# AsherBond/0-kno-vectorx

Measured on AMD Instinct MI355X. Metric: header_range_256 proofs/sec, higher is better.
Workload: dtype u64 (Goldilocks) / u8 (hashes)

## Files before the change

0-kno-vectorx_amd/csrc/vx_core.hip:

```cpp
#include <stdarg.h>
#include <stdlib.h>
#include <stdio.h>

#include "gl.cuh"
#include <dlfcn.h>

#include "vx_internal.h"

__attribute__((constructor)) static void vx_runtime_env() { setenv("GPU_MAX_HW_QUEUES", "16", 0); }

int32_t vx_fail(vx_ctx* ctx, int32_t code, const char* fmt, ...) {
    char buf[512];
    va_list ap;
    va_start(ap, fmt);
    vsnprintf(buf, sizeof buf, fmt, ap);
    va_end(ap);
    if (ctx) ctx->err = buf;
    return code;
}

static int32_t make_powtab(vx_ctx* ctx, uint64_t base, PowTab* out) {
    std::vector<uint64_t> h(3 * 2048);
    uint64_t b = base;
    for (int l = 0; l < 3; ++l) {
        uint64_t acc = 1;
        for (int j = 0; j < 2048; ++j) {
            h[l * 2048 + j] = acc;
            acc = glh::mul(acc, b);
        }
        b = glh::pow(b, 2048);
    }
    VX_HIP(hipMalloc(&out->d, h.size() * 8));
    VX_HIP(hipMemcpyAsync(out->d, h.data(), h.size() * 8, hipMemcpyHostToDevice, ctx->stream));
    VX_HIP(hipStreamSynchronize(ctx->stream));
    return VX_OK;
}

int32_t vx_get_shift_tab(vx_ctx* ctx, uint64_t base, PowTab* out) {
    auto it = ctx->shift_tabs.find(base);
    if (it == ctx->shift_tabs.end()) {
        PowTab t;
        VX_TRY(make_powtab(ctx, base, &t));
        it = ctx->shift_tabs.emplace(base, t).first;
    }
    *out = it->second;
    return VX_OK;
}

int32_t vx_get_tw2(vx_ctx* ctx, int log_s, int inverse, Tw2* out) {
    const int lo_bits = (log_s + 1) / 2, hi_bits = log_s - lo_bits;
    const int key = log_s * 2 + (inverse ? 1 : 0);
    auto it = ctx->tw2.find(key);
    if (it == ctx->tw2.end()) {
        const size_t nlo = (size_t)1 << lo_bits, nhi = (size_t)1 << hi_bits;
        std::vector<uint64_t> h(nlo + nhi);
        uint64_t w = glh::root(log_s);
        if (inverse) w = glh::inv(w);
        uint64_t acc = 1;
        for (size_t j = 0; j < nlo; ++j) {
            h[j] = acc;
            acc = glh::mul(acc, w);
        }
        const uint64_t wh = acc;
        acc = 1;
        for (size_t j = 0; j < nhi; ++j) {
            h[nlo + j] = acc;
            acc = glh::mul(acc, wh);
        }
        uint64_t* d = nullptr;
        VX_HIP(hipMalloc(&d, h.size() * 8));
        VX_HIP(hipMemcpyAsync(d, h.data(), h.size() * 8, hipMemcpyHostToDevice, ctx->stream));
        VX_HIP(hipStreamSynchronize(ctx->stream));
        it = ctx->tw2.emplace(key, d).first;
    }
    out->lo = it->second;
    out->hi = it->second + ((size_t)1 << lo_bits);
    out->lo_bits = lo_bits;
    return VX_OK;
}

void vx_pool_trim(vx_ctx* ctx) {
    (void)hipStreamSynchronize(ctx->stream);
    for (auto& kv : ctx->pool_free)
        for (void* p : kv.second) (void)hipFree(p);
    ctx->pool_free.clear();
}
void* vx_pool_alloc(vx_ctx* ctx, size_t bytes) {
    const size_t gran = (size_t)2 << 20;
    const size_t sz = ((bytes ? bytes : 1) + gran - 1) / gran * gran;
    auto it = ctx->pool_free.find(sz);
    void* p = nullptr;
    if (it != ctx->pool_free.end() && !it->second.empty()) {
        p = it->second.back();
        it->second.pop_back();
    } else if (hipMalloc(&p, sz) != hipSuccess) {
        (void)hipGetLastError();
        vx_pool_trim(ctx);
        if (hipMalloc(&p, sz) != hipSuccess) {
            (void)hipGetLastError();
            return nullptr;
        }
    }
    ctx->pool_live[p] = sz;
    return p;
}
void vx_pool_free(vx_ctx* ctx, void* p) {
    if (!p) return;
    auto it = ctx->pool_live.find(p);
    if (it == ctx->pool_live.end()) {
        (void)hipFree(p);
        return;
    }
    ctx->pool_free[it->second].push_back(p);
    ctx->pool_live.erase(it);
}

int32_t vx_scratch(vx_ctx* ctx, size_t n, uint64_t** out) {
    if (ctx->scratch_n < n) {
        if (ctx->scratch) {
            vx_pool_free(ctx, ctx->scratch);
            ctx->scratch = nullptr;
            ctx->scratch_n = 0;
        }
        ctx->scratch = (uint64_t*)vx_pool_alloc(ctx, n * 8);
        if (!ctx->scratch) return vx_fail(ctx, VX_ERR_OOM, "scratch: cannot allocate %zu bytes", n * 8);
        ctx->scratch_n = n;
    }
    *out = ctx->scratch;
    return VX_OK;
}

extern "C" {

const char* vx_backend_name(void) { return "hip-gfx950"; }

static thread_local int g_side_ctx = 0;
int32_t vx_ctx_create(int device, vx_ctx** out) {
    if (!out) return VX_ERR_ARG;
    *out = nullptr;
    int n_dev = 0;
    if (hipGetDeviceCount(&n_dev) != hipSuccess || n_dev == 0 || device < 0 || device >= n_dev) return VX_ERR_DEVICE;
    vx_ctx* ctx = new vx_ctx();
    ctx->device = device;
    ctx->scratch = nullptr;
    ctx->scratch_n = 0;
    ctx->pinned = nullptr;
    ctx->pinned_n = 0;
    {
        const char* sm = getenv("VX_SYNC_MODE");
        const char m = sm ? sm[0] : 'b';
        (void)hipSetDevice(device);
        (void)hipSetDeviceFlags(m == 's' ? hipDeviceScheduleSpin : m == 'y' ? hipDeviceScheduleYield : hipDeviceScheduleBlockingSync);
        (void)hipGetLastError();
    }
    hipError_t se = hipSetDevice(device);
    if (se == hipSuccess) {
        const char* sp = getenv("VX_STREAM_PRIO");
        int least = 0, greatest = 0;
        if (sp && sp[0] == '1' && hipDeviceGetStreamPriorityRange(&least, &greatest) == hipSuccess && least != greatest)
            se = hipStreamCreateWithPriority(&ctx->stream, hipStreamDefault, g_side_ctx ? least : greatest);
        else se = hipStreamCreate(&ctx->stream);
    }
    if (se != hipSuccess ||
        hipEventCreate(&ctx->ev0) != hipSuccess || hipEventCreate(&ctx->ev1) != hipSuccess) {
        delete ctx;
        return VX_ERR_DEVICE;
    }
    int32_t rc = make_powtab(ctx, glh::ROOT_2_32, &ctx->tw_fwd);
    if (rc == VX_OK) rc = make_powtab(ctx, glh::inv(glh::ROOT_2_32), &ctx->tw_inv);
    if (rc == VX_OK) {
        std::vector<uint64_t> f(2048), b(2048);
        uint64_t w = glh::root(12), wi = glh::inv(w), a = 1, c = 1;
        for (int j = 0; j < 2048; ++j) {
            f[j] = a;
            b[j] = c;
            a = glh::mul(a, w);
            c = glh::mul(c, wi);
        }
        if (hipMalloc(&ctx->w12_fwd, 2048 * 8) != hipSuccess || hipMalloc(&ctx->w12_inv, 2048 * 8) != hipSuccess ||
            hipMemcpy(ctx->w12_fwd, f.data(), 2048 * 8, hipMemcpyHostToDevice) != hipSuccess ||
            hipMemcpy(ctx->w12_inv, b.data(), 2048 * 8, hipMemcpyHostToDevice) != hipSuccess)
            rc = VX_ERR_DEVICE;
    }
    if (rc == VX_OK) {
        ctx->pinned_n = 1 << 20;
        if (hipHostMalloc(&ctx->pinned, ctx->pinned_n) != hipSuccess) rc = VX_ERR_DEVICE;
    }
    if (rc != VX_OK) {
        delete ctx;
        return rc;
    }
    *out = ctx;
    return VX_OK;
}

int32_t vx_ctx_destroy(vx_ctx* ctx) {
    if (!ctx) return VX_ERR_ARG;
    if (ctx->side) {
        vx_ctx_destroy(ctx->side);
        ctx->side = nullptr;
    }
    hipSetDevice(ctx->device);
    hipStreamSynchronize(ctx->stream);
    for (auto& kv : ctx->shift_tabs) hipFree(kv.second.d);
    for (auto& kv : ctx->periodic_cache) hipFree(kv.second);
    for (auto& kv : ctx->tw2) hipFree(kv.second);
    hipFree(ctx->tw_fwd.d);
    hipFree(ctx->tw_inv.d);
    hipFree(ctx->w12_fwd);
    hipFree(ctx->w12_inv);
    if (ctx->scratch) vx_pool_free(ctx, ctx->scratch);
    vx_pool_trim(ctx);
    for (auto& kv : ctx->pool_live) hipFree(kv.first);
    if (ctx->pinned) hipHostFree(ctx->pinned);
    hipEventDestroy(ctx->ev0);
    hipEventDestroy(ctx->ev1);
    hipStreamDestroy(ctx->stream);
    delete ctx;
    return VX_OK;
}

int32_t vx_sync(vx_ctx* ctx) {
    if (!ctx) return VX_ERR_ARG;
    VX_HIP(hipStreamSynchronize(ctx->stream));
    return VX_OK;
}
const char* vx_last_error(const vx_ctx* ctx) { return ctx ? ctx->err.c_str() : "null ctx"; }

int32_t vx_timer_start(vx_ctx* ctx) {
    if (!ctx) return VX_ERR_ARG;
    VX_HIP(hipEventRecord(ctx->ev0, ctx->stream));
    return VX_OK;
}
int32_t vx_timer_stop(vx_ctx* ctx, float* ms) {
    if (!ctx || !ms) return VX_ERR_ARG;
    VX_HIP(hipEventRecord(ctx->ev1, ctx->stream));
    VX_HIP(hipEventSynchronize(ctx->ev1));
    VX_HIP(hipEventElapsedTime(ms, ctx->ev0, ctx->ev1));
    return VX_OK;
}

int32_t vx_alloc(vx_ctx* ctx, size_t n, vx_buf** out) {
    if (!ctx || !out) return VX_ERR_ARG;
    VX_CHECK(n > 0, "vx_alloc: n == 0");
    vx_buf* b = new vx_buf{nullptr, n};
    b->d = (uint64_t*)vx_pool_alloc(ctx, n * 8);
    if (!b->d) {
        delete b;
        return vx_fail(ctx, VX_ERR_OOM, "device allocation of %zu bytes failed", n * 8);
    }
    *out = b;
    return VX_OK;
}
int32_t vx_free(vx_ctx* ctx, vx_buf* buf) {
    if (!ctx || !buf) return VX_ERR_ARG;
    vx_pool_free(ctx, buf->d);
    delete buf;
    return VX_OK;
}
int32_t vx_upload(vx_ctx* ctx, vx_buf* dst, size_t off, const uint64_t* src, size_t n) {
    if (!ctx || !dst || !src) return VX_ERR_ARG;
    VX_CHECK(off + n <= dst->n, "vx_upload: range [%zu,%zu) exceeds buffer of %zu", off, off + n, dst->n);
    VX_HIP(hipMemcpyAsync(dst->d + off, src, n * 8, hipMemcpyHostToDevice, ctx->stream));
    VX_HIP(hipStreamSynchronize(ctx->stream));
    return VX_OK;
}
int32_t vx_download(vx_ctx* ctx, const vx_buf* src, size_t off, uint64_t* dst, size_t n) {
    if (!ctx || !dst || !src) return VX_ERR_ARG;
    VX_CHECK(off + n <= src->n, "vx_download: range [%zu,%zu) exceeds buffer of %zu", off, off + n, src->n);
    VX_HIP(hipMemcpyAsync(dst, src->d + off, n * 8, hipMemcpyDeviceToHost, ctx->stream));
    VX_HIP(hipStreamSynchronize(ctx->stream));
    return VX_OK;
}
int32_t vx_copy(vx_ctx* ctx, vx_buf* dst, size_t doff, const vx_buf* src, size_t soff, size_t n) {
    if (!ctx || !dst || !src) return VX_ERR_ARG;
    VX_CHECK(doff + n <= dst->n && soff + n <= src->n, "vx_copy: out of range");
    VX_HIP(hipMemcpyAsync(dst->d + doff, src->d + soff, n * 8, hipMemcpyDeviceToDevice, ctx->stream));
    return VX_OK;
}
void* vx_buf_devptr(const vx_buf* buf) { return buf ? buf->d : nullptr; }
size_t vx_buf_len(const vx_buf* buf) { return buf ? buf->n : 0; }
}

__global__ void k_fill_random(uint64_t* d, size_t n, uint64_t seed) {
    size_t i = blockIdx.x * (size_t)blockDim.x + threadIdx.x;
    size_t stride = (size_t)gridDim.x * blockDim.x;
    for (; i < n; i += stride) {
        uint64_t z = seed + 0x9E3779B97F4A7C15ULL * (i + 1);
        z = (z ^ (z >> 30)) * 0xBF58476D1CE4E5B9ULL;
        z = (z ^ (z >> 27)) * 0x94D049BB133111EBULL;
        z ^= z >> 31;
        d[i] = gl_canon(z);
    }
}
template <int OP>
__global__ void k_batch(const uint64_t* a, const uint64_t* b, uint64_t* o, size_t n) {
    size_t i = blockIdx.x * (size_t)blockDim.x + threadIdx.x;
    size_t stride = (size_t)gridDim.x * blockDim.x;
    for (; i < n; i += stride) {
        uint64_t x = a[i], y = OP == 3 ? 0 : b[i], r;
        if (OP == 0) r = gl_add(x, y);
        else if (OP == 1) r = gl_sub(x, y);
        else if (OP == 2) r = gl_mul(x, y);
        else r = x ? gl_inv(x) : 0;
        o[i] = r;
    }
}
__global__ void k_ext_mul(const uint64_t* a, const uint64_t* b, uint64_t* o, size_t n) {
    size_t i = blockIdx.x * (size_t)blockDim.x + threadIdx.x;
    size_t stride = (size_t)gridDim.x * blockDim.x;
    for (; i < n; i += stride) {
        gl2 x{a[2 * i], a[2 * i + 1]}, y{b[2 * i], b[2 * i + 1]};
        gl2 r = gl2_mul(x, y);
        o[2 * i] = r.a;
        o[2 * i + 1] = r.b;
    }
}
static inline unsigned grid_for(size_t n) {
    size_t g = (n + 255) / 256;
    return (unsigned)(g < 1 ? 1 : (g > 2048 ? 2048 : g));
}
template <int OP>
static int32_t batch_op(vx_ctx* ctx, const vx_buf* a, const vx_buf* b, vx_buf* o, size_t n) {
    if (!ctx || !a || !o || (OP != 3 && !b)) return VX_ERR_ARG;
    VX_CHECK(n <= a->n && n <= o->n && (OP == 3 || n <= b->n), "batch op: n exceeds a buffer");
    if (n == 0) return VX_OK;
    hipLaunchKernelGGL(k_batch<OP>, dim3(grid_for(n)), dim3(256), 0, ctx->stream, a->d, OP == 3 ? a->d : b->d, o->d, n);
    VX_HIP(hipGetLastError());
    return VX_OK;
}
extern "C" {
int32_t vx_fill_random(vx_ctx* ctx, vx_buf* dst, size_t off, size_t n, uint64_t seed) {
    if (!ctx || !dst) return VX_ERR_ARG;
    VX_CHECK(off + n <= dst->n, "vx_fill_random: out of range");
    if (n == 0) return VX_OK;
    hipLaunchKernelGGL(k_fill_random, dim3(grid_for(n)), dim3(256), 0, ctx->stream, dst->d + off, n, seed);
    VX_HIP(hipGetLastError());
    return VX_OK;
}
int32_t vx_field_batch_add(vx_ctx* c, const vx_buf* a, const vx_buf* b, vx_buf* o, size_t n) { return batch_op<0>(c, a, b, o, n); }
int32_t vx_field_batch_sub(vx_ctx* c, const vx_buf* a, const vx_buf* b, vx_buf* o, size_t n) { return batch_op<1>(c, a, b, o, n); }
int32_t vx_field_batch_mul(vx_ctx* c, const vx_buf* a, const vx_buf* b, vx_buf* o, size_t n) { return batch_op<2>(c, a, b, o, n); }
int32_t vx_field_batch_inv(vx_ctx* c, const vx_buf* a, vx_buf* o, size_t n) { return batch_op<3>(c, a, nullptr, o, n); }
int32_t vx_ext_batch_mul(vx_ctx* ctx, const vx_buf* a, const vx_buf* b, vx_buf* o, size_t n) {
    if (!ctx || !a || !b || !o) return VX_ERR_ARG;
    VX_CHECK(2 * n <= a->n && 2 * n <= b->n && 2 * n <= o->n, "ext batch mul: n exceeds a buffer");
    if (n == 0) return VX_OK;
    hipLaunchKernelGGL(k_ext_mul, dim3(grid_for(n)), dim3(256), 0, ctx->stream, a->d, b->d, o->d, n);
    VX_HIP(hipGetLastError());
    return VX_OK;
}

int32_t vx_gather_proofs(vx_ctx* ctx, void* nccl_comm, int world, const uint64_t* mine, size_t n_words, uint64_t* out) {
    if (!ctx || !nccl_comm || !mine || !out || world < 1) return VX_ERR_ARG;
    typedef int (*all_gather_fn)(const void*, void*, size_t, int, void*, hipStream_t);
    static all_gather_fn all_gather = nullptr;
    if (!all_gather) all_gather = (all_gather_fn)dlsym(RTLD_DEFAULT, "ncclAllGather");
    if (!all_gather) {
        for (const char* name : {"librccl.so.1", "librccl.so"}) {
            void* h = dlopen(name, RTLD_NOLOAD | RTLD_LAZY);
            if (h && (all_gather = (all_gather_fn)dlsym(h, "ncclAllGather"))) break;
        }
    }
    if (!all_gather) return vx_fail(ctx, VX_ERR_DEVICE, "gather: ncclAllGather is not loaded in this process");
    if (n_words == 0) return VX_OK;
    uint64_t* sc;
    VX_TRY(vx_scratch(ctx, n_words * ((size_t)world + 1), &sc));
    VX_HIP(hipMemcpyAsync(sc, mine, n_words * 8, hipMemcpyHostToDevice, ctx->stream));
    const int rc = all_gather(sc, sc + n_words, n_words, 5, nccl_comm, ctx->stream);
    if (rc != 0) return vx_fail(ctx, VX_ERR_DEVICE, "gather: ncclAllGather failed (%d)", rc);
    VX_HIP(hipMemcpyAsync(out, sc + n_words, n_words * 8 * (size_t)world, hipMemcpyDeviceToHost, ctx->stream));
    VX_HIP(hipStreamSynchronize(ctx->stream));
    return VX_OK;
}
}

vx_ctx* vx_side_ctx(vx_ctx* ctx) {
    if (!ctx->side) {
        g_side_ctx = 1;
        if (vx_ctx_create(ctx->device, &ctx->side) != VX_OK) ctx->side = nullptr;
        g_side_ctx = 0;
    }
    return ctx->side;
}
```

0-kno-vectorx_amd/csrc/vx_internal.h:

```cpp
#pragma once
#include <hip/hip_runtime.h>
#include <stdint.h>
#include <map>
#include <string>
#include <vector>

#pragma GCC visibility push(default)
#include "../../include/vx.h"
#pragma GCC visibility pop
#include "glh.h"

#ifndef VX_TAIL_PRIO
#define VX_TAIL_PRIO 1
#endif
#if VX_TAIL_PRIO
#define VX_TAIL_KERNEL_ENTRY() __builtin_amdgcn_s_setprio(3)
#else
#define VX_TAIL_KERNEL_ENTRY() ((void)0)
#endif

struct vx_buf {
    uint64_t* d;
    size_t n;
};

struct PowTab {
    uint64_t* d;
};

struct vx_ctx {
    int device;
    hipStream_t stream;
    hipEvent_t ev0, ev1;
    std::string err;
    PowTab tw_fwd, tw_inv;
    uint64_t *w12_fwd, *w12_inv;
    std::map<uint64_t, PowTab> shift_tabs;
    std::map<int, uint64_t*> tw2;
    uint64_t* scratch;
    size_t scratch_n;
    void* pinned;
    size_t pinned_n;
    std::map<size_t, std::vector<void*>> pool_free;
    std::map<void*, size_t> pool_live;
    vx_ctx* side = nullptr;
    std::map<uint64_t, uint64_t*> periodic_cache;
};
vx_ctx* vx_side_ctx(vx_ctx* ctx);
void* vx_pool_alloc(vx_ctx* ctx, size_t bytes);
void vx_pool_free(vx_ctx* ctx, void* p);
void vx_pool_trim(vx_ctx* ctx);
int32_t vx_fail(vx_ctx* ctx, int32_t code, const char* fmt, ...);

struct Scratch {
    vx_ctx* ctx = nullptr;
    uint64_t* base = nullptr;
    size_t words = 0;
    hipError_t err = hipSuccess;
    std::vector<std::pair<uint64_t**, size_t>> regions;
    Scratch() = default;
    Scratch(const Scratch&) = delete;
    Scratch& operator=(const Scratch&) = delete;
    ~Scratch() {
        if (base) vx_pool_free(ctx, base);
    }
    void add(uint64_t*& p, size_t n) { regions.push_back({&p, words}), words += n; }
    void alloc(vx_ctx* c) {
        ctx = c, base = (uint64_t*)vx_pool_alloc(c, words * 8);
        for (auto& r : regions) *r.first = base ? base + r.second : nullptr;
    }
    bool ok() const { return base && err == hipSuccess; }
    void keep(hipError_t e) {
        if (err == hipSuccess) err = e;
    }
    void copy(void* dst, const void* src, size_t bytes, hipMemcpyKind kind) {
        if (ok()) err = hipMemcpyAsync(dst, src, bytes, kind, ctx->stream);
    }
    void up(void* dst, const void* src, size_t bytes) { copy(dst, src, bytes, hipMemcpyHostToDevice); }
    void down(void* dst, const void* src, size_t bytes) { copy(dst, src, bytes, hipMemcpyDeviceToHost); }
    void fill(void* dst, int byte, size_t bytes) {
        if (ok()) err = hipMemsetAsync(dst, byte, bytes, ctx->stream);
    }
    void launched() { keep(hipGetLastError()); }
    void sync() {
        if (ok()) err = hipStreamSynchronize(ctx->stream);
    }
    int32_t status(const char* what) const {
        if (!base) return vx_fail(ctx, VX_ERR_OOM, "%s: out of device memory", what);
        return err == hipSuccess ? VX_OK : vx_fail(ctx, VX_ERR_DEVICE, "%s: %s", what, hipGetErrorString(err));
    }
};

struct vx_tree {
    uint64_t* levels;
    size_t n_leaves;
    int cap_height;
    size_t total;
};

#define VX_HIP(call)                                                                              \
    do {                                                                                          \
        hipError_t e_ = (call);                                                                   \
        if (e_ != hipSuccess)                                                                     \
            return vx_fail(ctx, e_ == hipErrorOutOfMemory ? VX_ERR_OOM : VX_ERR_DEVICE, "%s: %s", \
                           #call, hipGetErrorString(e_));                                         \
    } while (0)
#define VX_CHECK(cond, ...)                                   \
    do {                                                      \
        if (!(cond)) return vx_fail(ctx, VX_ERR_ARG, __VA_ARGS__); \
    } while (0)
#define VX_TRY(call)            \
    do {                        \
        int32_t r_ = (call);    \
        if (r_ != VX_OK) return r_; \
    } while (0)

int32_t vx_get_shift_tab(vx_ctx* ctx, uint64_t base, PowTab* out);
int32_t vx_scratch(vx_ctx* ctx, size_t n_u64, uint64_t** out);
int32_t vx_merkle_build_dev(vx_ctx* ctx, const uint64_t* data, size_t n_leaves, size_t leaf_len, int layout,
                            int cap_height, vx_tree** out);

int32_t vx_ntt_dev(vx_ctx* ctx, uint64_t* d, int log_n, size_t n_cols, size_t col_stride, int inverse, uint64_t shift, int order);
int32_t vx_lde_dev(vx_ctx* ctx, const uint64_t* src, int log_n, size_t n_cols, int rate_bits, uint64_t shift, int src_kind,
                   uint64_t* dst, uint64_t* coeffs_out);
int32_t vx_gather_rows_dev(vx_ctx* ctx, const uint64_t* lde, int log_N, size_t n_cols, const uint64_t* leaf_idx, size_t n_idx,
                           uint64_t* out);
void vx_gather_rows_enqueue(vx_ctx* ctx, const uint64_t* lde, int log_N, size_t n_cols, const uint64_t* idx_d, size_t n_idx, uint64_t* out_d);
void vx_merkle_open_enqueue(vx_ctx* ctx, const vx_tree* tree, const uint64_t* idx_d, size_t n_idx, uint64_t* out_d);
void vx_fri_leaves_enqueue(vx_ctx* ctx, const uint64_t* evals, int log_n, int arity_bits, const uint64_t* idx_d, size_t n_idx, uint64_t* out_d);
int32_t vx_fri_fold_dev(vx_ctx* ctx, const uint64_t* evals, int log_n, int arity_bits, const uint64_t beta[2], uint64_t shift,
                        uint64_t* out);
int32_t vx_fri_layer_tree_dev(vx_ctx* ctx, const uint64_t* evals, int log_n, int arity_bits, int cap_height, vx_tree** out);
int32_t vx_fri_leaves_dev(vx_ctx* ctx, const uint64_t* evals, int log_n, int arity_bits, const uint64_t* leaf_idx, size_t n_idx,
                          uint64_t* out);

struct Tw2 {
    const uint64_t* lo;
    const uint64_t* hi;
    int lo_bits;
};
int32_t vx_get_tw2(vx_ctx* ctx, int log_s, int inverse, Tw2* out);
int32_t vx_lde_consume_dev(vx_ctx* ctx, uint64_t* values, int log_n, size_t n_cols, int rate_bits, uint64_t shift, uint64_t* dst);
struct vx_chal_hook {
    int32_t (*fn)(void* user, const uint64_t* pub, size_t n_pub, const uint64_t* cap, size_t cap_words, uint64_t* chal, size_t n_chal);
    void* user;
};
int32_t vx_stark_prove_impl(vx_ctx* ctx, int air_id, const vx_stark_config* cfg, uint64_t* trace_d, size_t trace_len, int consume_trace,
                            int log_n, const uint64_t* public_inputs, size_t n_public, uint64_t* proof_out, size_t proof_cap,
                            size_t* proof_len, const vx_chal_hook* hook = nullptr);
void vx_shared_challenges_n(const uint64_t* const* pubs, const size_t* n_pubs, const uint64_t* const* caps, size_t k, size_t cap_words, uint64_t* out, size_t n_out);
void vx_shared_challenges(const uint64_t* pub_a, size_t n_a, const uint64_t* cap_a, const uint64_t* pub_b, size_t n_b, const uint64_t* cap_b,
                          size_t cap_words, uint64_t* out, size_t n_out);
int32_t vx_stark_verify_ext(const vx_stark_config* cfg, const uint64_t* proof, size_t proof_len, int expect_air, const uint64_t* expect_public,
                            size_t n_expect_public, const uint64_t* ext_chal, const uint64_t** apub_out, int* log_n_out, char* err, size_t errlen);
int32_t vx_lde_keep_dev(vx_ctx* ctx, const uint64_t* values, int log_n, size_t n_cols, int rate_bits, uint64_t shift, uint64_t* coef_brev,
                        uint64_t* dst);
int32_t vx_scan_cols_dev(vx_ctx* ctx, uint64_t* data, int log_n, size_t n_cols, uint64_t* totals_host);
int32_t vx_sha_tree_trace_dev(vx_ctx* ctx, const uint8_t* state_roots, const uint8_t* data_roots, size_t n_leaves, int log_tree, uint64_t* trace_d,
                              uint64_t pub_out[17]);
int32_t vx_bus_close_dev(vx_ctx* ctx, uint64_t* z_cols, int log_n, uint64_t aux_pub[2]);
int32_t vx_ed_trace_dev(vx_ctx* ctx, const uint8_t* pubkeys, const uint8_t* sigs, const uint8_t* msg, uint32_t msg_len, const uint8_t* signed_flags, size_t n_sigs,
                        int log_n, uint64_t bus_on, uint64_t* trace_d, uint64_t pub_out[2]);
int32_t vx_sha512_trace_dev(vx_ctx* ctx, const uint8_t* pubkeys, const uint8_t* sigs, const uint8_t* msg, const uint8_t* flags, size_t n_sigs, int log_n, uint64_t bus_on,
                            uint64_t* trace_d, uint64_t pub_out[15]);
int32_t vx_epoch_end_trace_dev(vx_ctx* ctx, const uint8_t* header_d, size_t header_bytes, uint32_t start_position, uint32_t num_authorities, uint64_t bus_on, uint64_t* trace_d,
                               uint64_t pub_out[10], uint32_t* window_length_out);
int32_t vx_sha_chain_trace_dev(vx_ctx* ctx, const uint8_t* pubkeys, size_t n_keys, const uint8_t* signed_flags, uint64_t bus_on, int log_n, uint64_t* trace_d,
                               uint64_t public_inputs_out[10], uint8_t commitment_out[32]);
int32_t vx_merkle_open_trace_dev(vx_ctx* ctx, const vx_tree* tree, const uint64_t* leaf_idx, size_t n_idx, int log_n, uint64_t* trace_d, uint64_t pub_out[9]);
void vx_merkle_levels_launch(vx_ctx* ctx, uint64_t* levels, size_t n_leaves, size_t cap);
```

0-kno-vectorx_amd/csrc/vx_poseidon.hip:

```cpp
#include "poseidon.cuh"
#include "poseidon_air.cuh"
#include "vx_internal.h"

__global__ __launch_bounds__(256) void k_poseidon_batch(uint64_t* states, size_t n) {
    size_t i = blockIdx.x * (size_t)blockDim.x + threadIdx.x;
    if (i >= n) return;
    uint64_t s[12];
#pragma unroll
    for (int k = 0; k < 12; ++k) s[k] = states[12 * i + k];
    poseidon_permute(s);
#pragma unroll
    for (int k = 0; k < 12; ++k) states[12 * i + k] = s[k];
}

#ifndef VX_HASH_WAVES
#define VX_HASH_WAVES 6
#endif
template <int LAYOUT>
__global__ __launch_bounds__(256) __attribute__((amdgpu_waves_per_eu(VX_HASH_WAVES, 8))) void k_hash_leaves(const uint64_t* data, size_t n_leaves, int log_n, size_t leaf_len,
                                                     uint64_t* digests) {
    size_t p = blockIdx.x * (size_t)blockDim.x + threadIdx.x;
    if (p >= n_leaves) return;
    const size_t estride = LAYOUT == VX_LEAVES_ROW_MAJOR ? 1 : n_leaves;
    const uint64_t* src = LAYOUT == VX_LEAVES_ROW_MAJOR ? data + p * leaf_len : data + p;
    size_t j = LAYOUT == VX_LEAVES_COLS_BITREV ? brev32((uint32_t)p, log_n) : p;
    uint64_t s[12];
#pragma unroll
    for (int k = 0; k < 12; ++k) s[k] = 0;
    if (leaf_len <= 4) {
        for (size_t e = 0; e < leaf_len; ++e) s[e] = src[e * estride];
    } else {
        size_t e = 0;
        for (; e + 8 < leaf_len; e += 8) {
#pragma unroll
            for (int k = 0; k < 8; ++k) s[k] = src[(e + k) * estride];
            poseidon_permute<false>(s);
        }
#pragma unroll
        for (int k = 0; k < 8; ++k)
            if (e + k < leaf_len) s[k] = src[(e + k) * estride];
        poseidon_permute(s);
    }
    uint64_t* d = digests + 4 * j;
    d[0] = s[0];
    d[1] = s[1];
    d[2] = s[2];
    d[3] = s[3];
}

template <int LAYOUT>
__global__ __launch_bounds__(256) void k_hash_leaves_coop(const uint64_t* data, size_t n_leaves, int log_n, size_t leaf_len,
                                                          uint64_t* digests) {
    VX_TAIL_KERNEL_ENTRY();
    __shared__ uint64_t lds[16 * 12];
    const int l = threadIdx.x & 15, grp = threadIdx.x >> 4;
    uint64_t* g = lds + 12 * grp;
    const size_t t = blockIdx.x * (size_t)16 + grp;
    const size_t p = t < n_leaves ? t : n_leaves - 1;
    const size_t estride = LAYOUT == VX_LEAVES_ROW_MAJOR ? 1 : n_leaves;
    const uint64_t* src = LAYOUT == VX_LEAVES_ROW_MAJOR ? data + p * leaf_len : data + p;
    const size_t j = LAYOUT == VX_LEAVES_COLS_BITREV ? brev32((uint32_t)p, log_n) : p;
    uint64_t s = 0;
    if (leaf_len <= 4) {
        if ((size_t)l < leaf_len) s = src[(size_t)l * estride];
    } else {
        for (size_t e = 0; e < leaf_len; e += 8) {
            if (l < 8 && e + l < leaf_len) s = src[(e + l) * estride];
            s = poseidon_permute_coop<false>(s, l, g);
        }
        s = gl_canon(s);
    }
    if (l < 4 && t < n_leaves) digests[4 * j + l] = s;
}
#ifndef VX_TOP_THREADS
#define VX_TOP_THREADS 256
#endif
#ifndef VX_TOP_LANE_MIN
#define VX_TOP_LANE_MIN 32
#endif
constexpr int TOP_MAX_S = 9, TOP_GROUPS = VX_TOP_THREADS / 16;
static_assert(VX_TOP_THREADS >= (1 << (TOP_MAX_S - 1)) && VX_TOP_THREADS <= 1024, "one lane per parent of the widest level");
__global__ __launch_bounds__(VX_TOP_THREADS) void k_merkle_top(uint64_t* levels, size_t off, size_t cur, int s) {
    VX_TAIL_KERNEL_ENTRY();
    __shared__ uint64_t buf[2][4 << (TOP_MAX_S - 1)];
    __shared__ uint64_t xch[12 * TOP_GROUPS];
    const int tid = threadIdx.x, l = tid & 15, grp = tid >> 4;
    const uint64_t* child_g = levels + off + 4 * ((size_t)blockIdx.x << s);
    for (int j = 1; j <= s; ++j) {
        const int np = 1 << (s - j);
        off += 4 * cur;
        cur >>= 1;
        uint64_t* parent_g = levels + off + 4 * ((size_t)blockIdx.x << (s - j));
        uint64_t* parent_l = buf[j & 1];
        const uint64_t* child_l = buf[(j - 1) & 1];
        if (VX_TOP_LANE_MIN <= 256 && np >= VX_TOP_LANE_MIN) {
            if (tid < np) {
                uint64_t st[12];
#pragma unroll
                for (int k = 0; k < 8; ++k) st[k] = j == 1 ? child_g[8 * tid + k] : child_l[8 * tid + k];
                st[8] = st[9] = st[10] = st[11] = 0;
                poseidon_permute(st);
#pragma unroll
                for (int k = 0; k < 4; ++k) parent_l[4 * tid + k] = parent_g[4 * tid + k] = st[k];
            }
        } else {
            for (int base = 0; base < np; base += TOP_GROUPS) {
                const int t = base + grp, i = t < np ? t : np - 1;
                uint64_t x = 0;
                if (l < 8) x = j == 1 ? child_g[8 * i + l] : child_l[8 * i + l];
                x = poseidon_permute_coop(x, l, xch + 12 * grp);
                if (l < 4 && t < np) parent_l[4 * i + l] = parent_g[4 * i + l] = x;
            }
        }
        __syncthreads();
    }
}
constexpr size_t COOP_MAX_LEAVES = 16384;

__global__ __launch_bounds__(256) void k_merkle_level(const uint64_t* child, uint64_t* parent, size_t n_parent) {
    size_t i = blockIdx.x * (size_t)blockDim.x + threadIdx.x;
    if (i >= n_parent) return;
    uint64_t s[12];
#pragma unroll
    for (int k = 0; k < 8; ++k) s[k] = child[8 * i + k];
    s[8] = s[9] = s[10] = s[11] = 0;
    poseidon_permute(s);
    parent[4 * i] = s[0];
    parent[4 * i + 1] = s[1];
    parent[4 * i + 2] = s[2];
    parent[4 * i + 3] = s[3];
}

__global__ void k_gather_siblings(const uint64_t* levels, size_t n_leaves, int depth, const uint64_t* idx, size_t n_idx,
                                  uint64_t* out) {
    VX_TAIL_KERNEL_ENTRY();
    size_t t = blockIdx.x * (size_t)blockDim.x + threadIdx.x;
    if (t >= n_idx * depth) return;
    size_t k = t / depth;
    int lvl = (int)(t - k * depth);
    size_t off = 0, cur = n_leaves;
    for (int l = 0; l < lvl; ++l) {
        off += 4 * cur;
        cur >>= 1;
    }
    size_t node = (idx[k] >> lvl) ^ 1;
    for (int e = 0; e < 4; ++e) out[4 * t + e] = levels[off + 4 * node + e];
}


__global__ __launch_bounds__(256) void k_poseidon_air_trace(const uint64_t* in, size_t n_perm, uint64_t* tr) {
    const size_t p = blockIdx.x * (size_t)256 + threadIdx.x;
    if (p >= n_perm) return;
    uint64_t s[12];
#pragma unroll
    for (int i = 0; i < 12; ++i) s[i] = gl_canon(in[12 * p + i]);
    poseidon_air_walk(s, tr, 32 * n_perm, 32 * p);
}

void vx_merkle_levels_launch(vx_ctx* ctx, uint64_t* levels, size_t n_leaves, size_t cap) {
    size_t off = 0, cur = n_leaves;
    while (cur > cap && (cur >> 1) > COOP_MAX_LEAVES) {
        const size_t np = cur >> 1;
        hipLaunchKernelGGL(k_merkle_level, dim3((unsigned)((np + 255) / 256)), dim3(256), 0, ctx->stream, levels + off, levels + off + 4 * cur, np);
        off += 4 * cur;
        cur = np;
    }
    int todo = 0;
    while ((cap << todo) < cur) ++todo;
    while (todo > 0) {
        const int s = todo < TOP_MAX_S ? todo : TOP_MAX_S;
        hipLaunchKernelGGL(k_merkle_top, dim3((unsigned)(cur >> s)), dim3(VX_TOP_THREADS), 0, ctx->stream, levels, off, cur, s);
        for (int j = 0; j < s; ++j) {
            off += 4 * cur;
            cur >>= 1;
        }
        todo -= s;
    }
}

void vx_merkle_open_enqueue(vx_ctx* ctx, const vx_tree* tree, const uint64_t* idx_d, size_t n_idx, uint64_t* out_d) {
    int log_n = 0;
    while (((size_t)1 << log_n) < tree->n_leaves) ++log_n;
    const int depth = log_n - tree->cap_height;
    const size_t tot = n_idx * depth;
    if (tot == 0) return;
    hipLaunchKernelGGL(k_gather_siblings, dim3((unsigned)((tot + 255) / 256)), dim3(256), 0, ctx->stream, tree->levels,
                       tree->n_leaves, depth, idx_d, n_idx, out_d);
}

int32_t vx_merkle_build_dev(vx_ctx* ctx, const uint64_t* data, size_t n_leaves, size_t leaf_len, int layout,
                            int cap_height, vx_tree** out) {
    int log_n = 0;
    while (((size_t)1 << log_n) < n_leaves) ++log_n;
    VX_CHECK(((size_t)1 << log_n) == n_leaves, "merkle: n_leaves %zu is not a power of two", n_leaves);
    VX_CHECK(cap_height >= 0 && cap_height <= log_n, "merkle: cap_height %d > log2(n_leaves) %d", cap_height, log_n);
    VX_CHECK(leaf_len >= 1, "merkle: empty leaves");
    size_t total = 0, cur = n_leaves, cap = (size_t)1 << cap_height;
    while (cur > cap) {
        total += 4 * cur;
        cur >>= 1;
    }
    total += 4 * cur;
    vx_tree* t = new vx_tree{nullptr, n_leaves, cap_height, total};
    t->levels = (uint64_t*)vx_pool_alloc(ctx, total * 8);
    if (!t->levels) {
        delete t;
        return vx_fail(ctx, VX_ERR_OOM, "merkle: cannot allocate %zu bytes", total * 8);
    }
    unsigned g = (unsigned)((n_leaves + 255) / 256);
    if (n_leaves <= COOP_MAX_LEAVES && leaf_len > 4) {
        const unsigned gc = (unsigned)((n_leaves + 15) / 16);
        if (layout == VX_LEAVES_ROW_MAJOR)
            hipLaunchKernelGGL(k_hash_leaves_coop<VX_LEAVES_ROW_MAJOR>, dim3(gc), dim3(256), 0, ctx->stream, data, n_leaves, log_n, leaf_len, t->levels);
        else if (layout == VX_LEAVES_COLS_BITREV)
            hipLaunchKernelGGL(k_hash_leaves_coop<VX_LEAVES_COLS_BITREV>, dim3(gc), dim3(256), 0, ctx->stream, data, n_leaves, log_n, leaf_len, t->levels);
        else
            hipLaunchKernelGGL(k_hash_leaves_coop<VX_LEAVES_COLS>, dim3(gc), dim3(256), 0, ctx->stream, data, n_leaves, log_n, leaf_len, t->levels);
    } else if (layout == VX_LEAVES_ROW_MAJOR)
        hipLaunchKernelGGL(k_hash_leaves<VX_LEAVES_ROW_MAJOR>, dim3(g), dim3(256), 0, ctx->stream, data, n_leaves, log_n, leaf_len, t->levels);
    else if (layout == VX_LEAVES_COLS_BITREV)
        hipLaunchKernelGGL(k_hash_leaves<VX_LEAVES_COLS_BITREV>, dim3(g), dim3(256), 0, ctx->stream, data, n_leaves, log_n, leaf_len, t->levels);
    else
        hipLaunchKernelGGL(k_hash_leaves<VX_LEAVES_COLS>, dim3(g), dim3(256), 0, ctx->stream, data, n_leaves, log_n, leaf_len, t->levels);
    vx_merkle_levels_launch(ctx, t->levels, n_leaves, cap);
    hipError_t le = hipGetLastError();
    if (le != hipSuccess) {
        vx_pool_free(ctx, t->levels);
        delete t;
        return vx_fail(ctx, VX_ERR_DEVICE, "merkle launch: %s", hipGetErrorString(le));
    }
    *out = t;
    return VX_OK;
}

extern "C" {
int32_t vx_poseidon_permute_batch(vx_ctx* ctx, vx_buf* states, size_t n) {
    if (!ctx || !states) return VX_ERR_ARG;
    VX_CHECK(12 * n <= states->n, "poseidon batch: %zu states exceed the buffer", n);
    if (n == 0) return VX_OK;
    hipLaunchKernelGGL(k_poseidon_batch, dim3((unsigned)((n + 255) / 256)), dim3(256), 0, ctx->stream, states->d, n);
    VX_HIP(hipGetLastError());
    return VX_OK;
}
int32_t vx_poseidon_air_trace(vx_ctx* ctx, const vx_buf* states, size_t n_perm, vx_buf* trace_out) {
    if (!ctx || !states || !trace_out) return VX_ERR_ARG;
    VX_CHECK(n_perm >= 1 && (n_perm & (n_perm - 1)) == 0 && n_perm <= ((size_t)1 << 22), "poseidon air trace: %zu permutations (a power of two, at most 2^22)", n_perm);
    VX_CHECK(12 * n_perm <= states->n && 48 * 32 * n_perm <= trace_out->n, "poseidon air trace: buffers too small");
    hipLaunchKernelGGL(k_poseidon_air_trace, dim3((unsigned)((n_perm + 255) / 256)), dim3(256), 0, ctx->stream, states->d, n_perm, trace_out->d);
    VX_HIP(hipGetLastError());
    return VX_OK;
}
int32_t vx_merkle_build(vx_ctx* ctx, const vx_buf* data, size_t off, size_t n_leaves, size_t leaf_len, int layout,
                        int cap_height, vx_tree** out) {
    if (!ctx || !data || !out) return VX_ERR_ARG;
    VX_CHECK(layout >= 0 && layout <= 2, "merkle: bad layout %d", layout);
    VX_CHECK(off + n_leaves * leaf_len <= data->n, "merkle: %zu leaves x %zu exceed the buffer", n_leaves, leaf_len);
    return vx_merkle_build_dev(ctx, data->d + off, n_leaves, leaf_len, layout, cap_height, out);
}
int32_t vx_merkle_free(vx_ctx* ctx, vx_tree* tree) {
    if (!ctx || !tree) return VX_ERR_ARG;
    vx_pool_free(ctx, tree->levels);
    delete tree;
    return VX_OK;
}
int32_t vx_merkle_cap(vx_ctx* ctx, const vx_tree* tree, uint64_t* cap_out) {
    if (!ctx || !tree || !cap_out) return VX_ERR_ARG;
    size_t cap = (size_t)4 << tree->cap_height;
    VX_HIP(hipMemcpyAsync(cap_out, tree->levels + tree->total - cap, cap * 8, hipMemcpyDeviceToHost, ctx->stream));
    VX_HIP(hipStreamSynchronize(ctx->stream));
    return VX_OK;
}
int32_t vx_merkle_leaf_digests(vx_ctx* ctx, const vx_tree* tree, uint64_t* out) {
    if (!ctx || !tree || !out) return VX_ERR_ARG;
    VX_HIP(hipMemcpyAsync(out, tree->levels, tree->n_leaves * 32, hipMemcpyDeviceToHost, ctx->stream));
    VX_HIP(hipStreamSynchronize(ctx->stream));
    return VX_OK;
}
int32_t vx_merkle_open(vx_ctx* ctx, const vx_tree* tree, const uint64_t* leaf_idx, size_t n_idx, uint64_t* siblings_out) {
    if (!ctx || !tree || !leaf_idx || !siblings_out) return VX_ERR_ARG;
    int log_n = 0;
    while (((size_t)1 << log_n) < tree->n_leaves) ++log_n;
    int depth = log_n - tree->cap_height;
    for (size_t i = 0; i < n_idx; ++i) VX_CHECK(leaf_idx[i] < tree->n_leaves, "merkle open: index out of range");
    if (depth == 0 || n_idx == 0) return VX_OK;
    uint64_t* sc;
    size_t tot = n_idx * depth;
    VX_TRY(vx_scratch(ctx, n_idx + 4 * tot, &sc));
    VX_HIP(hipMemcpyAsync(sc, leaf_idx, n_idx * 8, hipMemcpyHostToDevice, ctx->stream));
    vx_merkle_open_enqueue(ctx, tree, sc, n_idx, sc + n_idx);
    VX_HIP(hipGetLastError());
    VX_HIP(hipMemcpyAsync(siblings_out, sc + n_idx, 4 * tot * 8, hipMemcpyDeviceToHost, ctx->stream));
    VX_HIP(hipStreamSynchronize(ctx->stream));
    return VX_OK;
}
}
```

Baseline: 8.550.

## Add persistent resident-block leaf hashing with atomic tile counter for large Merkle builds

Adds a persistent-kernel variant of leaf hashing: a grid sized to a fixed number of blocks per compute unit pulls 256-leaf tiles from a global atomic counter until all tiles are done. A padded shared-memory array caps how many blocks fit on each compute unit, and the waves-per-EU attribute is pinned to match. It is used only when the leaf-hash permutation count reaches a threshold. The aim is to cut per-block launch and tail overhead and to keep occupancy controlled. In exchange it adds an extra memset, an atomic and two barriers per tile, and occupancy is lower than the grid kernel.

```diff
diff --git a/0-kno-vectorx_amd/csrc/vx_core.hip b/0-kno-vectorx_amd/csrc/vx_core.hip
--- a/0-kno-vectorx_amd/csrc/vx_core.hip
+++ b/0-kno-vectorx_amd/csrc/vx_core.hip
@@ -183,6 +183,13 @@
             rc = VX_ERR_DEVICE;
     }
     if (rc == VX_OK) {
+        hipDeviceProp_t prop;
+        if (hipGetDeviceProperties(&prop, device) != hipSuccess || prop.multiProcessorCount < 1 ||
+            hipMalloc(&ctx->hash_next_tile, sizeof(unsigned)) != hipSuccess)
+            rc = VX_ERR_DEVICE;
+        else ctx->n_cus = prop.multiProcessorCount;
+    }
+    if (rc == VX_OK) {
         ctx->pinned_n = 1 << 20;
         if (hipHostMalloc(&ctx->pinned, ctx->pinned_n) != hipSuccess) rc = VX_ERR_DEVICE;
     }
@@ -209,6 +216,7 @@
     hipFree(ctx->tw_inv.d);
     hipFree(ctx->w12_fwd);
     hipFree(ctx->w12_inv);
+    hipFree(ctx->hash_next_tile);
     if (ctx->scratch) vx_pool_free(ctx, ctx->scratch);
     vx_pool_trim(ctx);
     for (auto& kv : ctx->pool_live) hipFree(kv.first);
diff --git a/0-kno-vectorx_amd/csrc/vx_internal.h b/0-kno-vectorx_amd/csrc/vx_internal.h
--- a/0-kno-vectorx_amd/csrc/vx_internal.h
+++ b/0-kno-vectorx_amd/csrc/vx_internal.h
@@ -45,6 +45,8 @@
     std::map<void*, size_t> pool_live;
     vx_ctx* side = nullptr;
     std::map<uint64_t, uint64_t*> periodic_cache;
+    int n_cus = 0;
+    unsigned* hash_next_tile = nullptr;
 };
 vx_ctx* vx_side_ctx(vx_ctx* ctx);
 void* vx_pool_alloc(vx_ctx* ctx, size_t bytes);
diff --git a/0-kno-vectorx_amd/csrc/vx_poseidon.hip b/0-kno-vectorx_amd/csrc/vx_poseidon.hip
--- a/0-kno-vectorx_amd/csrc/vx_poseidon.hip
+++ b/0-kno-vectorx_amd/csrc/vx_poseidon.hip
@@ -17,10 +17,7 @@
 #define VX_HASH_WAVES 6
 #endif
 template <int LAYOUT>
-__global__ __launch_bounds__(256) __attribute__((amdgpu_waves_per_eu(VX_HASH_WAVES, 8))) void k_hash_leaves(const uint64_t* data, size_t n_leaves, int log_n, size_t leaf_len,
-                                                     uint64_t* digests) {
-    size_t p = blockIdx.x * (size_t)blockDim.x + threadIdx.x;
-    if (p >= n_leaves) return;
+__device__ __forceinline__ void hash_leaf(const uint64_t* data, size_t n_leaves, int log_n, size_t leaf_len, uint64_t* digests, size_t p) {
     const size_t estride = LAYOUT == VX_LEAVES_ROW_MAJOR ? 1 : n_leaves;
     const uint64_t* src = LAYOUT == VX_LEAVES_ROW_MAJOR ? data + p * leaf_len : data + p;
     size_t j = LAYOUT == VX_LEAVES_COLS_BITREV ? brev32((uint32_t)p, log_n) : p;
@@ -47,6 +44,38 @@
     d[2] = s[2];
     d[3] = s[3];
 }
+template <int LAYOUT>
+__global__ __launch_bounds__(256) __attribute__((amdgpu_waves_per_eu(VX_HASH_WAVES, 8))) void k_hash_leaves(const uint64_t* data, size_t n_leaves, int log_n, size_t leaf_len,
+                                                     uint64_t* digests) {
+    size_t p = blockIdx.x * (size_t)blockDim.x + threadIdx.x;
+    if (p >= n_leaves) return;
+    hash_leaf<LAYOUT>(data, n_leaves, log_n, leaf_len, digests, p);
+}
+
+#ifndef VX_HASH_RESIDENT
+#define VX_HASH_RESIDENT 4
+#endif
+#if VX_HASH_RESIDENT
+static_assert(VX_HASH_RESIDENT >= 1 && VX_HASH_RESIDENT <= 8, "blocks of four waves per compute unit: 1..8");
+constexpr unsigned HASH_PAD_WORDS = (160 / (VX_HASH_RESIDENT + 1) + 1) * 1024 / 4;
+static_assert((size_t)HASH_PAD_WORDS * 4 * (VX_HASH_RESIDENT + 1) > 160 * 1024 && (size_t)HASH_PAD_WORDS * 4 * VX_HASH_RESIDENT <= 160 * 1024,
+              "the pad admits W blocks per compute unit and not W + 1");
+template <int LAYOUT>
+__global__ __launch_bounds__(256) __attribute__((amdgpu_waves_per_eu(VX_HASH_RESIDENT, VX_HASH_RESIDENT))) void k_hash_leaves_resident(
+    const uint64_t* data, size_t n_leaves, int log_n, size_t leaf_len, uint64_t* digests, unsigned* next_tile, unsigned tiles) {
+    __shared__ unsigned pad[HASH_PAD_WORDS];
+    if (leaf_len == 0) pad[1 + threadIdx.x] = (unsigned)n_leaves;
+    for (;;) {
+        if (threadIdx.x == 0) pad[0] = atomicAdd(next_tile, 1u);
+        __syncthreads();
+        const unsigned tile = pad[0];
+        __syncthreads();
+        if (tile >= tiles) return;
+        const size_t p = tile * (size_t)256 + threadIdx.x;
+        if (p < n_leaves) hash_leaf<LAYOUT>(data, n_leaves, log_n, leaf_len, digests, p);
+    }
+}
+#endif
 
 template <int LAYOUT>
 __global__ __launch_bounds__(256) void k_hash_leaves_coop(const uint64_t* data, size_t n_leaves, int log_n, size_t leaf_len,
@@ -116,6 +145,13 @@
     }
 }
 constexpr size_t COOP_MAX_LEAVES = 16384;
+#ifndef VX_HASH_RESIDENT_MIN_PERMS
+#define VX_HASH_RESIDENT_MIN_PERMS ((size_t)1 << 22)
+#endif
+#ifndef VX_HASH_GRID_FORCE
+#define VX_HASH_GRID_FORCE 0
+#endif
+[[maybe_unused]] constexpr size_t HASH_RESIDENT_MIN_PERMS = VX_HASH_RESIDENT_MIN_PERMS;
 
 __global__ __launch_bounds__(256) void k_merkle_level(const uint64_t* child, uint64_t* parent, size_t n_parent) {
     size_t i = blockIdx.x * (size_t)blockDim.x + threadIdx.x;
@@ -208,6 +244,11 @@
         return vx_fail(ctx, VX_ERR_OOM, "merkle: cannot allocate %zu bytes", total * 8);
     }
     unsigned g = (unsigned)((n_leaves + 255) / 256);
+#if VX_HASH_RESIDENT
+    const bool resident = leaf_len <= 4 ? HASH_RESIDENT_MIN_PERMS == 0 : n_leaves * ((leaf_len + 7) / 8) >= HASH_RESIDENT_MIN_PERMS;
+#else
+    const bool resident = false;
+#endif
     if (n_leaves <= COOP_MAX_LEAVES && leaf_len > 4) {
         const unsigned gc = (unsigned)((n_leaves + 15) / 16);
         if (layout == VX_LEAVES_ROW_MAJOR)
@@ -216,6 +257,23 @@
             hipLaunchKernelGGL(k_hash_leaves_coop<VX_LEAVES_COLS_BITREV>, dim3(gc), dim3(256), 0, ctx->stream, data, n_leaves, log_n, leaf_len, t->levels);
         else
             hipLaunchKernelGGL(k_hash_leaves_coop<VX_LEAVES_COLS>, dim3(gc), dim3(256), 0, ctx->stream, data, n_leaves, log_n, leaf_len, t->levels);
+    } else if (resident) {
+#if VX_HASH_RESIDENT
+        const unsigned room = (unsigned)VX_HASH_RESIDENT * (unsigned)ctx->n_cus;
+        const unsigned gr = VX_HASH_GRID_FORCE ? (unsigned)VX_HASH_GRID_FORCE : g < room ? g : room;
+        hipError_t ze = hipMemsetAsync(ctx->hash_next_tile, 0, sizeof(unsigned), ctx->stream);
+        if (ze != hipSuccess) {
+            vx_pool_free(ctx, t->levels);
+            delete t;
+            return vx_fail(ctx, VX_ERR_DEVICE, "merkle tile counter: %s", hipGetErrorString(ze));
+        }
+        if (layout == VX_LEAVES_ROW_MAJOR)
+            hipLaunchKernelGGL(k_hash_leaves_resident<VX_LEAVES_ROW_MAJOR>, dim3(gr), dim3(256), 0, ctx->stream, data, n_leaves, log_n, leaf_len, t->levels, ctx->hash_next_tile, g);
+        else if (layout == VX_LEAVES_COLS_BITREV)
+            hipLaunchKernelGGL(k_hash_leaves_resident<VX_LEAVES_COLS_BITREV>, dim3(gr), dim3(256), 0, ctx->stream, data, n_leaves, log_n, leaf_len, t->levels, ctx->hash_next_tile, g);
+        else
+            hipLaunchKernelGGL(k_hash_leaves_resident<VX_LEAVES_COLS>, dim3(gr), dim3(256), 0, ctx->stream, data, n_leaves, log_n, leaf_len, t->levels, ctx->hash_next_tile, g);
+#endif
     } else if (layout == VX_LEAVES_ROW_MAJOR)
         hipLaunchKernelGGL(k_hash_leaves<VX_LEAVES_ROW_MAJOR>, dim3(g), dim3(256), 0, ctx->stream, data, n_leaves, log_n, leaf_len, t->levels);
     else if (layout == VX_LEAVES_COLS_BITREV)
```

Result: faster. 8.652, median of 6 (+1.2%).
